# tum-pbs/differentiable-piso

Hardware: AMD Instinct MI355X
Metric: PISO steps/s (fwd+adjoint) at 2048^2 staggered grid (higher is better)
Workload: dtype f64

## Files before the change

### differentiable-piso_amd/csrc/cg.hip

```cpp
#include <atomic>
#include "cg_kernels.h"
#include "cg_dispatch.h"
#include "cg_tiny.h"
#include "options.h"
#include <cstdio>
#include <vector>

namespace piso {

struct CgProfile {
  int enabled = 0, stride = 8;
  double ms[4] = {0, 0, 0, 0};
  long long count[4] = {0, 0, 0, 0};
};
static CgProfile g_prof;

struct HostPoll {
  CgState* pinned = nullptr;
  hipEvent_t ev[2] = {nullptr, nullptr};
  hipEvent_t seg_ev[2] = {nullptr, nullptr};
  int cus = 0;
};
static std::atomic<unsigned> g_persist_launches{0};
static int g_persist_fallbacks = 0;
static thread_local int tl_xcd_map[kPersistMaxGrid];
static thread_local int tl_xcd_map_n = 0;
static long long g_tiny_solves = 0;
enum { DI_PATH = 0, DI_SIZEOF_T, DI_SIZEOF_CT, DI_V, DI_RECON, DI_SYMMETRIC, DI_ROWS_PER_WAVE, DI_K1_GRID, DI_K1_TILES, DI_R, DI_NQ,
       DI_WAVES, DI_LAUNCH_GRID, DI_PADDED, DI_XCD_LOCAL, DI_FELL_BACK, DI_TINY_PER_X, DI_K2_GRID, DI_SEGMENTS, DI_COUNT };
static thread_local int tl_dispatch[DI_COUNT];
static thread_local int tl_dispatch_n = 0;
static bool g_xcd_local_failed = false;
static long long g_verify_runs = 0;
static int g_verify_failures = 0;
constexpr int kPollDevices = 16;
static thread_local HostPoll tl_poll_dev[kPollDevices];
static thread_local HostPoll* tl_poll_cur = &tl_poll_dev[0];
#define tl_poll (*tl_poll_cur)

static int ensure_poll() {
  int dev = 0;
  PISO_HIP_CHECK(hipGetDevice(&dev));
  if (dev < 0 || dev >= kPollDevices) { set_error_msg("piso_cg_solve: device ordinal out of range"); return PISO_ERR_INVALID_ARG; }
  tl_poll_cur = &tl_poll_dev[dev];
  if (!tl_poll.pinned) {
    PISO_HIP_CHECK(hipHostMalloc(reinterpret_cast<void**>(&tl_poll.pinned), 2 * sizeof(CgState), hipHostMallocDefault));
    PISO_HIP_CHECK(hipEventCreateWithFlags(&tl_poll.ev[0], hipEventDisableTiming));
    PISO_HIP_CHECK(hipEventCreateWithFlags(&tl_poll.ev[1], hipEventDisableTiming));
    PISO_HIP_CHECK(hipDeviceGetAttribute(&tl_poll.cus, hipDeviceAttributeMultiprocessorCount, dev));
  }
  return PISO_OK;
}

constexpr size_t kPadMaxCells = (size_t)1 << 19;
static bool padded_dims(int nx, int ny, int per_x, int per_y, int elem, int* nxp, int* nyp) {
  *nxp = nx; *nyp = ny;
  if (elem != 8 || nx % 2 != 0 || nx < 8 || ny < 8) return false;
  const bool pad_x = nx % 128 != 0, pad_y = ny % 2 != 0;
  if (!pad_x && !pad_y) return false;
  const int px = (nx + 127) / 128 * 128;
  int py = (ny + 3) / 4 * 4;
  if (px != nx && per_x) return false;
  if (py != ny && per_y) {
    py = ny;
    if (ny % 2 != 0 || ((long long)(px / 128) * (ny / 2)) % 2 != 0) return false;
  }
  if ((size_t)px * py > kPadMaxCells) return false;
  *nxp = px; *nyp = py;
  return true;
}

template <typename T>
static size_t cg_workspace_bytes(int nx_in, int ny_in) {
  int nx = nx_in, ny = ny_in;
  const bool padded = padded_dims(nx_in, ny_in, 0, 0, (int)sizeof(T), &nx, &ny);
  const size_t n = (size_t)nx * ny + (padded ? 2 * (size_t)nx * ny : 0);
  size_t b = 0;
  b += 11 * align_up(n * sizeof(T), 256);
  b += align_up(4 * n * sizeof(float), 256) + 256;
  b += 3 * align_up(3 * kMaxPartials * sizeof(T), 256);
  b += align_up(SC_COUNT * sizeof(T), 256) + align_up(2 * sizeof(CgState), 256) + 512;
  b += align_up(kPersistWsWordsAll * sizeof(unsigned), 256);
  return b + 4096;
}

static void record_dispatch(int path, size_t state_bytes, size_t coef_bytes, int tiny_per_x, int V = 0, bool recon = false, bool symmetric = false,
                            const CgTiling* t = nullptr, const PersistPlan* p = nullptr, bool fell_back = false) {
  int* d = tl_dispatch;
  for (int i = 0; i < DI_COUNT; ++i) d[i] = 0;
  d[DI_PATH] = path; d[DI_SIZEOF_T] = (int)state_bytes; d[DI_SIZEOF_CT] = (int)coef_bytes; d[DI_TINY_PER_X] = tiny_per_x;
  d[DI_V] = V; d[DI_RECON] = recon ? 1 : 0; d[DI_SYMMETRIC] = symmetric ? 1 : 0; d[DI_FELL_BACK] = fell_back ? 1 : 0;
  if (t) { d[DI_ROWS_PER_WAVE] = t->rows_per_wave; d[DI_K1_GRID] = t->g1; d[DI_K1_TILES] = t->k1_tiles; d[DI_K2_GRID] = t->g2; }
  if (p) d[DI_PADDED] = p->ragged ? 1 : 0;
  if (p && p->R) { d[DI_R] = p->R; d[DI_NQ] = p->NQ; d[DI_WAVES] = p->waves; d[DI_LAUNCH_GRID] = p->launch_grid; d[DI_XCD_LOCAL] = p->xcd_local ? 1 : 0; }
  tl_dispatch_n = DI_COUNT;
}

struct EventPool {
  static constexpr int kMax = 64;
// ... 11 lines not shown
      PISO_HIP_CHECK(hipEventCreate(&ep.start[q][i]));
      PISO_HIP_CHECK(hipEventCreate(&ep.stop[q][i]));
    }
  ep.created = true;
  return PISO_OK;
}

static int read_profile(const EventPool& ep, const SegmentTimes& seg, float* kernel_ms_out) {
  double ms[2] = {0, 0};
  for (int q = 0; q < 2; ++q)
    for (int i = 0; i < ep.used[q]; ++i) {
      float t = 0;
      PISO_HIP_CHECK(hipEventElapsedTime(&t, ep.start[q][i], ep.stop[q][i]));
      ms[q] += t;
    }
  if (kernel_ms_out) {
    kernel_ms_out[0] = ep.used[0] ? (float)(ms[0] / ep.used[0]) : 0.f;
    kernel_ms_out[1] = ep.used[1] ? (float)(ms[1] / ep.used[1]) : 0.f;
  }
  if (g_prof.enabled) {
    for (int q = 0; q < 2; ++q) { g_prof.ms[q] += ms[q]; g_prof.count[q] += ep.used[q]; }
    g_prof.ms[2] += seg.ms; g_prof.count[2] += seg.iters; g_prof.count[3] += seg.launches;
  }
  if (kernel_ms_out && seg.iters > 0) { kernel_ms_out[0] = (float)(seg.ms / seg.iters); kernel_ms_out[1] = 0.f; }
  return PISO_OK;
}

struct PersistTiming {
  unsigned long long* ticks = nullptr;
  ~PersistTiming() { if (ticks) (void)hipFree(ticks); }
};
static int print_persist_timing(const unsigned long long* ticks, int grid, int k_last) {
  std::vector<unsigned long long> h(12 * grid);
  PISO_HIP_CHECK(hipMemcpy(h.data(), ticks, h.size() * sizeof(unsigned long long), hipMemcpyDeviceToHost));
  const char* names[9] = {"D (p update, stencil, sums, publish)", "exchange", "U (stencil, x / r update, ring)", "-", "-",
                           "  exchange: wave sums + drain of the perimeter stores", "  exchange: first barrier", "  exchange: publish + polling",
                           "  exchange: record sums + second barrier"};
  const double f = 0.01 / (double)(k_last > 0 ? k_last : 1);
  if (opt(OPT_CG_PERSIST_TIMING) >= 2) {
    for (int b = 0; b < grid; ++b)
      fprintf(stderr, "cg_persist_wg %3d xcd %d band %3d  D %.2f  exchange %.2f  U %.2f  | drain %.2f  barrier1 %.2f  publish+poll %.2f  sums %.2f\n", b, (int)h[9 * grid + b], (int)h[10 * grid + b],
              f * (double)h[0 * grid + b], f * (double)h[1 * grid + b], f * (double)h[2 * grid + b],
              f * (double)h[5 * grid + b], f * (double)h[6 * grid + b], f * (double)h[7 * grid + b], f * (double)h[8 * grid + b]);
  }
  for (int q = 0; q < 9; ++q) {
    double s = 0, mn = 1e300, mx = 0;
    for (int b = 0; b < grid; ++b) { const double v = (double)h[q * grid + b]; s += v; mn = v < mn ? v : mn; mx = v > mx ? v : mx; }
    fprintf(stderr, "cg_persist %s: avg %.2f us/iter  min %.2f  max %.2f\n", names[q], f * s / grid, f * mn, f * mx);
  }
  return PISO_OK;
}

template <typename T, typename CT>
static int verify_residual(const CgArgs<T>& a, const PersistCtl& pc, hipStream_t stream, bool* failed) {
  unsigned* out2 = reinterpret_cast<unsigned*>(pc.err) + 4;
  PISO_HIP_CHECK(hipMemsetAsync(out2, 0, 2 * sizeof(unsigned), stream));
  const int gvf = grid_for((long long)a.nx * a.ny, kBlock * 4, 1024);
  cg_verify_sum_x<T><<<gvf, kBlock, 0, stream>>>(a, a.partsA);
  cg_verify_gap<T, CT><<<gvf, kBlock, 0, stream>>>(a, a.partsA, gvf, out2);
  PISO_LAUNCH_CHECK();
  unsigned h2[2] = {0, 0};
  PISO_HIP_CHECK(hipMemcpyAsync(h2, out2, sizeof(h2), hipMemcpyDeviceToHost, stream));
  PISO_HIP_CHECK(hipStreamSynchronize(stream));
  float gap, scale;
  memcpy(&gap, &h2[0], 4); memcpy(&scale, &h2[1], 4);
  ++g_verify_runs;
  *failed = (gap > 1e-5f * scale && gap > 1e-30f) || opt(OPT_CG_VERIFY) == 2;
  return PISO_OK;
}

static int inspect_poll(int slot, int* stop_it) {
  hipError_t e = hipEventSynchronize(tl_poll.ev[slot]);
  if (e != hipSuccess) { set_error("hipEventSynchronize", e); return -1; }
  if (tl_poll.pinned[slot].done) { *stop_it = tl_poll.pinned[slot].iterations; return 1; }
  return 0;
}
static int poll_batch(size_t n) {
  const double t_iter_us = (double)n * 120.0 / 4.0e6;
  const int batch = (int)(1000.0 / (t_iter_us < 8.0 ? 8.0 : t_iter_us));
  return batch < 10 ? 10 : (batch > 200 ? 200 : batch);
}

template <typename T, typename CT, int V, bool RECON>
static int cg_run(CgArgs<T> a, unsigned* persist_ws, bool symmetric, float accuracy, int max_iterations, int rank_deficient, int reset, int fixed,
                  int* iterations_out, float* kernel_ms_out, hipStream_t stream, bool allow_persist) {
  const size_t n = (size_t)a.nx * a.ny;
  const CgTiling tile = cg_tile(a, V, opt(OPT_CG_RPW), opt(OPT_CG_MAXBLOCKS));
  const int g1 = tile.g1, g2 = tile.g2, gflat = tile.gflat;
  a.accuracy = fixed ? -1.0f : accuracy;

  { const int rc = ensure_poll(); if (rc != PISO_OK) return rc; }
  const bool prof = (kernel_ms_out != nullptr) || g_prof.enabled;
  EventPool& ep = tl_events;
  if (prof) { const int rc = ensure_events(ep); if (rc != PISO_OK) return rc; }
  ep.used[0] = ep.used[1] = 0;
  const int prof_stride = g_prof.stride > 0 ? g_prof.stride : 8;

  cg_init<T><<<gflat, kBlock, 0, stream>>>(a, rank_deficient);
  PISO_LAUNCH_CHECK();

  const int batch = poll_batch(n);
  int sv = 0, polls = 0, stop_it = -1;
  const int total = fixed ? fixed : max_iterations;
  bool finished = false;
  bool pending = false;
  int k_last = -1;
  PersistPlan plan = persist_plan(PersistQuery{a.nx, a.ny, V, a.per_y, a.nx_true != 0, sizeof(T), sizeof(CT), RECON, symmetric, false, tl_poll.cus,
                                               opt(OPT_CG_PERSIST), opt(OPT_CG_PERSIST_R), opt(OPT_CG_PERSIST_HALF), opt(OPT_CG_PERSIST_NQ),
                                               opt(OPT_CG_XCD_LOCAL), g_xcd_local_failed, allow_persist});
  PersistCtl pc;
  { const int rc = persist_prepare<T, CT, RECON, false>(plan, tl_poll.cus, pc, persist_ws, stream); if (rc != PISO_OK) return rc; }
  PersistTiming timing;
  if (plan.R && kPersistDiag && opt_on(OPT_CG_PERSIST_TIMING)) {
    PISO_HIP_CHECK(hipMalloc(reinterpret_cast<void**>(&timing.ticks), 12 * plan.launch_grid * sizeof(unsigned long long)));
    PISO_HIP_CHECK(hipMemsetAsync(timing.ticks, 0, 12 * plan.launch_grid * sizeof(unsigned long long), stream));
    pc.timing = timing.ticks;
  }
  record_dispatch(plan.R ? 3 : 2, sizeof(T), sizeof(CT), 0, V, RECON, symmetric, &tile, &plan, !allow_persist);
  const int seg_len = persist_segment_len(n, opt(OPT_CG_SEGMENT));
  hipEvent_t* seg_ev = tl_poll.seg_ev;
  if (plan.R && prof && !seg_ev[0]) { PISO_HIP_CHECK(hipEventCreate(&seg_ev[0])); PISO_HIP_CHECK(hipEventCreate(&seg_ev[1])); }
  SegmentTimes seg;
  int segments_run = 0, unsynced = 0;
  for (int k = 0; k < total && !finished; ++k) {
    const bool is_reset = !fixed && ((k + 1) % reset == 0);
    if (plan.R && k > 0 && !is_reset) {
      int ke = total;
      if (!fixed) { const int next_reset = ((k + 1 + reset - 1) / reset) * reset - 1; if (next_reset < ke) ke = next_reset; }
      if (ke > k + seg_len) ke = k + seg_len;
      if (ke > k) {
        if (prof) PISO_HIP_CHECK(hipEventRecord(seg_ev[0], stream));
        { const int rc = persist_launch<T, CT, RECON, false>(plan, a, pc, g_persist_launches.fetch_add(1, std::memory_order_relaxed), k, ke, sv, pending, NoSlab{}, stream);
          if (rc != PISO_OK) return rc; }
        if (prof) PISO_HIP_CHECK(hipEventRecord(seg_ev[1], stream));
        const bool defer = !prof && ke - k <= 32 && unsynced + (ke - k) <= 256 && ke < total;
        unsynced = defer ? unsynced + (ke - k) : 0;
        if (!defer) {
          PISO_HIP_CHECK(hipMemcpyAsync(&tl_poll.pinned[0], &a.state[0], sizeof(CgState), hipMemcpyDeviceToHost, stream));
          int herr = 0;
          PISO_HIP_CHECK(hipMemcpyAsync(&herr, pc.err, sizeof(int), hipMemcpyDeviceToHost, stream));
          PISO_HIP_CHECK(hipStreamSynchronize(stream));
          if (herr) {
            ++g_persist_fallbacks;
            if (plan.xcd_local) g_xcd_local_failed = true;
            return kPersistRetry;
          }
          if (prof) {
            const int ran = tl_poll.pinned[0].done ? (tl_poll.pinned[0].iterations - k > 0 ? tl_poll.pinned[0].iterations - k : 0) : ke - k;
            float t = 0; PISO_HIP_CHECK(hipEventElapsedTime(&t, seg_ev[0], seg_ev[1])); seg.ms += t; seg.iters += ran < ke - k ? ran : ke - k; ++seg.launches;
          }
          if (tl_poll.pinned[0].done) { finished = true; stop_it = tl_poll.pinned[0].iterations; }
        }
        ++segments_run;
        k_last = ke - 1;
        pending = false;
        k = ke - 1;
        continue;
      }
    }
    const bool sample = prof && (k % prof_stride == prof_stride - 1) && ep.used[0] < EventPool::kMax && !is_reset && k > 0;
    if (is_reset) {
      if (pending) { cg_flush_x<T><<<gflat, kBlock, 0, stream>>>(a, k - 1, sv); pending = false; }
      cg_k1<T, CT, V, RECON><<<g1, kBlock, 0, stream>>>(a, k, MODE_RESET, sv, k > 0 ? 1 : 0, 0);
      ++sv;
      cg_reset_residual<T><<<gflat, kBlock, 0, stream>>>(a, sv);
      cg_k1<T, CT, V, RECON><<<g1, kBlock, 0, stream>>>(a, k, MODE_INIT, sv, 0, 0);
    } else if (k == 0) {
      cg_k1<T, CT, V, RECON><<<g1, kBlock, 0, stream>>>(a, k, MODE_INIT, sv, 0, 0);
    } else {
      if (sample) PISO_HIP_CHECK(hipEventRecord(ep.start[0][ep.used[0]], stream));
      cg_k1<T, CT, V, RECON><<<g1, kBlock, 0, stream>>>(a, k, MODE_NORMAL, sv, 1, pending ? 1 : 0);
      if (sample) PISO_HIP_CHECK(hipEventRecord(ep.stop[0][ep.used[0]++], stream));
      ++sv;
    }
    if (sample) PISO_HIP_CHECK(hipEventRecord(ep.start[1][ep.used[1]], stream));
    cg_k2<T, V><<<g2, kBlock, 0, stream>>>(a, k, sv);
    if (sample) PISO_HIP_CHECK(hipEventRecord(ep.stop[1][ep.used[1]++], stream));
    PISO_LAUNCH_CHECK();
    pending = true;
    k_last = k;
    if (!fixed && ((k + 1) % batch == 0) && k + 1 < total) {
      const int slot = polls & 1;
      PISO_HIP_CHECK(hipMemcpyAsync(&tl_poll.pinned[slot], &a.state[sv & 1], sizeof(CgState), hipMemcpyDeviceToHost, stream));
      PISO_HIP_CHECK(hipEventRecord(tl_poll.ev[slot], stream));
      if (polls > 0) {
        const int r = inspect_poll((polls - 1) & 1, &stop_it);
        if (r < 0) return PISO_ERR_HIP;
        if (r > 0) finished = true;
      }
      ++polls;
    }
  }
  if (pending && k_last >= 0) cg_flush_x<T><<<gflat, kBlock, 0, stream>>>(a, k_last, sv);
  if (!fixed && !finished) {
    const int slot = polls & 1;
    PISO_HIP_CHECK(hipMemcpyAsync(&tl_poll.pinned[slot], &a.state[sv & 1], sizeof(CgState), hipMemcpyDeviceToHost, stream));
    PISO_HIP_CHECK(hipEventRecord(tl_poll.ev[slot], stream));
    const int r = inspect_poll(slot, &stop_it);
    if (r < 0) return PISO_ERR_HIP;
    if (r > 0) finished = true;
  }
  PISO_HIP_CHECK(hipStreamSynchronize(stream));
  if (opt(OPT_CG_XCD_MAP) == 1) {
    tl_xcd_map_n = 0;
    if (segments_run > 0 && !plan.xcd_local && plan.grid <= kPersistMaxGrid) {
      PISO_HIP_CHECK(hipMemcpy(tl_xcd_map, pc.xcd + kPersistXcdTable, (size_t)plan.grid * sizeof(int), hipMemcpyDeviceToHost));
      tl_xcd_map_n = plan.grid;
    }
  }
  if (segments_run > 0) {
    int herr = 0;
    PISO_HIP_CHECK(hipMemcpy(&herr, pc.err, sizeof(int), hipMemcpyDeviceToHost));
    if (herr) { ++g_persist_fallbacks; return kPersistRetry; }
  }
  if (segments_run > 0 && sizeof(T) == 8 && !fixed && opt(OPT_CG_VERIFY) != 0) {
    bool failed = false;
    { const int rc = verify_residual<T, CT>(a, pc, stream, &failed); if (rc != PISO_OK) return rc; }
    if (failed) { ++g_verify_failures; ++g_persist_fallbacks; return kPersistRetry; }
  }
  if (timing.ticks) { const int rc = print_persist_timing(timing.ticks, plan.grid, k_last); if (rc != PISO_OK) return rc; }
  if (iterations_out) *iterations_out = finished ? stop_it : total;
  tl_dispatch[DI_SEGMENTS] = segments_run;
  return prof ? read_profile(ep, seg, kernel_ms_out) : PISO_OK;
}

template <typename T>
__global__ __launch_bounds__(kBlock) void cg_copy_rows(const T* __restrict__ src, T* __restrict__ dst, int nx, int ny, int ld_src, int ld_dst) {
  const size_t n = (size_t)nx * ny;
  for (size_t i = (size_t)blockIdx.x * kBlock + threadIdx.x; i < n; i += (size_t)gridDim.x * kBlock) {
    const size_t j = i / (size_t)nx, c = i % (size_t)nx;
    dst[j * (size_t)ld_dst + c] = src[j * (size_t)ld_src + c];
  }
}

template <typename T>
static int cg_solve(int nx, int ny, int per_x, int per_y, const T* L, const T* b, T* x_out, float accuracy,
                    int max_iterations, int rank_deficient, int reset, int fixed, int* iterations_out,
                    float* kernel_ms_out, void* ws, size_t ws_bytes, piso_stream_t stream_, int* iterations_dev = nullptr) {
  tl_dispatch_n = 0;
  if (nx < 1 || ny < 1 || !L || !b || !x_out || !ws || max_iterations < 0 || reset < 1) {
    set_error_msg("piso_cg_solve: invalid argument");
    return PISO_ERR_INVALID_ARG;
  }
  if (ws_bytes < cg_workspace_bytes<T>(nx, ny)) {
    set_error_msg("piso_cg_solve: workspace too small");
    return PISO_ERR_INVALID_ARG;
  }
  hipStream_t stream = static_cast<hipStream_t>(stream_);
  const size_t n_true = (size_t)nx * ny;
  if (n_true <= (size_t)kTinyMaxCells && opt(OPT_CG_TINY) != 0 && opt(OPT_CG_PERSIST) < 0) {
    CgState* st_dev = reinterpret_cast<CgState*>(ws);
    const int total = fixed ? fixed : max_iterations;
    hipEvent_t* ev = nullptr;
    if (kernel_ms_out) {
      { const int rc = ensure_poll(); if (rc != PISO_OK) return rc; }
      ev = tl_poll.seg_ev;
      if (!ev[0]) { PISO_HIP_CHECK(hipEventCreate(&ev[0])); PISO_HIP_CHECK(hipEventCreate(&ev[1])); }
      PISO_HIP_CHECK(hipEventRecord(ev[0], stream));
    }
    const bool async = iterations_dev != nullptr;
    const bool cols = nx <= 64 && ny <= kColsMaxNy && (!per_x || nx == 64) && opt(OPT_CG_TINY) != 2;
    if (cols && per_x)
      cg_tiny_cols<T, true><<<1, kTinyThreads, 0, stream>>>(L, b, x_out, nx, ny, per_y, fixed ? -1.0f : accuracy, total, fixed ? 0 : reset,
                                                            rank_deficient, st_dev, iterations_dev);
    else if (cols)
      cg_tiny_cols<T, false><<<1, kTinyThreads, 0, stream>>>(L, b, x_out, nx, ny, per_y, fixed ? -1.0f : accuracy, total, fixed ? 0 : reset,
                                                             rank_deficient, st_dev, iterations_dev);
    else
      cg_tiny<T><<<1, kTinyThreads, 0, stream>>>(L, b, x_out, nx, ny, per_x, per_y, fixed ? -1.0f : accuracy, total, fixed ? 0 : reset,
                                                 rank_deficient, st_dev, iterations_dev);
    PISO_LAUNCH_CHECK();
    ++g_tiny_solves;
// ... 173 lines not shown
```

### differentiable-piso_amd/csrc/cg_kernels.h

```cpp
#pragma once
#include <stdlib.h>

#include "piso_common.h"

namespace piso {

struct CgState {
  int flag;
  int done;
  int iterations;
  int pad;
};

enum { MODE_NORMAL = 0, MODE_INIT = 1, MODE_RESET = 2 };
enum { SC_C = 0, SC_PZ = 1, SC_VS = 2, SC_ALPHA = 3, SC_COUNT = 8 };

template <typename T>
struct CgArgs {
  const T* cC;
  const void *oS, *oW, *oE, *oN;
  const T* b;
  T *x, *r, *z;
  T* p[2];
  T* zp[2];
  T* partsA;
  T* partsB;
  T* partsS;
  T* scal;
  CgState* state;
  int nx, ny, per_x, per_y;
  const T* gA;
  const T* gB;
  int ntx, nty, rows_per_wave;
  int nA, nB;
  float accuracy;
  int nt;
  int nx_true, ny_true;
  double ncells;
};
template <typename T>
__device__ __forceinline__ bool true_cell(const CgArgs<T>& a, size_t i) {
  if (!a.nx_true) return true;
  return (int)(i % (size_t)a.nx) < a.nx_true && (int)(i / (size_t)a.nx) < a.ny_true;
}

template <typename T, int V>
struct Vec {
  T v[V];
};

template <typename S, int V>
__device__ __forceinline__ Vec<S, V> ldc(const S* __restrict__ p) {
  Vec<S, V> o;
  constexpr int B = sizeof(S) * V;
  using raw4 = __attribute__((ext_vector_type(4))) unsigned int;
  using raw2 = __attribute__((ext_vector_type(2))) unsigned int;
  if constexpr (B % 16 == 0) {
#pragma unroll
    for (int q = 0; q < B / 16; ++q) {
      const raw4 t = reinterpret_cast<const raw4*>(p)[q];
      __builtin_memcpy(reinterpret_cast<char*>(&o) + 16 * q, &t, 16);
    }
  } else if constexpr (B == 8) {
    const raw2 t = *reinterpret_cast<const raw2*>(p);
    __builtin_memcpy(&o, &t, 8);
  } else {
    static_assert(V == 1, "unsupported vector width");
    o.v[0] = p[0];
  }
  return o;
}
template <typename T, int V>
__device__ __forceinline__ Vec<T, V> ldv(const T* __restrict__ p) { return ldc<T, V>(p); }

template <typename S, int V>
__device__ __forceinline__ Vec<S, V> ldc_nt(const S* __restrict__ p) {
  Vec<S, V> o;
  constexpr int B = sizeof(S) * V;
  using raw4 = __attribute__((ext_vector_type(4))) unsigned int;
  using raw2 = __attribute__((ext_vector_type(2))) unsigned int;
  if constexpr (B % 16 == 0) {
#pragma unroll
    for (int q = 0; q < B / 16; ++q) {
      const raw4 t = __builtin_nontemporal_load(reinterpret_cast<const raw4*>(p) + q);
      __builtin_memcpy(reinterpret_cast<char*>(&o) + 16 * q, &t, 16);
    }
  } else if constexpr (B == 8) {
    const raw2 t = __builtin_nontemporal_load(reinterpret_cast<const raw2*>(p));
    __builtin_memcpy(&o, &t, 8);
  } else {
    o.v[0] = __builtin_nontemporal_load(p);
  }
// ... 93 lines not shown
    for (int e = 0; e < V; ++e) { o.s.v[e] = 0; o.q.v[e] = 0; }
    if (!active) return o;
    if (a.per_y != 2) {
      if (j < 0) { if (!a.per_y) return o; j = ny - 1; }
      if (j >= ny) { if (!a.per_y) return o; j = 0; }
    }
    const ptrdiff_t i = (ptrdiff_t)j * nx + c0;
    o.s = ldv<T, V>(src + i);
    if (use_pin) o.q = ldv<T, V>(pin + i);
    return o;
  };

  const CgState st = a.state[sv & 1];
  const T sc_pz = a.scal[SC_PZ], sc_vs = a.scal[SC_VS], sc_alpha = a.scal[SC_ALPHA];
  const int ntiles = a.ntx * a.nty;
  const XcdRange tr = xcd_range(ntiles);
  const int dir = (wave & 1) ? -1 : 1;
  auto tile_geom = [&](int t, int& jb, int& je, int& c0, bool& active) {
    const int ty = t / a.ntx, tx = t - ty * a.ntx;
    jb = (ty * 4 + wave) * a.rows_per_wave;
    je = min(jb + a.rows_per_wave, ny);
    c0 = (tx * 64 + lane) * V;
    active = c0 < nx;
  };
  Raw rawB, rawC;
  {
    int jb, je, c0; bool active;
    if (tr.begin < tr.end) {
      tile_geom(tr.begin, jb, je, c0, active);
      if (jb < ny) {
        const int j = (dir > 0) ? jb : je - 1;
        rawB = load_raw(j - dir, c0, active);
        rawC = load_raw(j, c0, active);
      }
    }
  }

  T beta = 0;
  CgState nst = st;
  if (do_check) {
    T pb[3];
    prologue_reduce<T, 3>(a.partsB, a.nB, a.gB, pb, smem);
    if (!st.done) {
      if (k > 0 && (k % 5) == 0) {
        const int exceeded = pb[2] > 0;
        if (st.flag && !exceeded) { nst.done = 1; nst.iterations = k; }
        else nst.flag = 1;
      }
      if (mode == MODE_NORMAL) beta = -(pb[0] + sc_vs * pb[1]) / sc_pz;
    }
  }
  if (mode == MODE_RESET && !nst.done) nst.flag = 0;
  if (writes_state && blockIdx.x == 0 && threadIdx.x == 0) a.state[(sv + 1) & 1] = nst;
  if (st.done) return;
  const T alpha_prev = pending ? sc_alpha : (T)0;
  const bool only_flush = nst.done;

  auto combine = [&](const Raw& w) -> Vec<T, V> {
    Vec<T, V> o = w.s;
    if (use_pin) {
#pragma unroll
      for (int e = 0; e < V; ++e) o.v[e] = fma(beta, w.q.v[e], o.v[e]);
    }
    return o;
  };
  auto val_at = [&](int j, int c) -> T {
    if (a.per_y != 2) {
      if (j < 0) { if (!a.per_y) return (T)0; j = ny - 1; }
      if (j >= ny) { if (!a.per_y) return (T)0; j = 0; }
    }
    const ptrdiff_t i = (ptrdiff_t)j * nx + c;
    T v = src[i];
    if (use_pin) v = fma(beta, pin[i], v);
    return v;
  };

  T acc_p = 0, acc_pr = 0, acc_pz = 0;
  for (int t = tr.begin; t < tr.end; t += tr.step) {
    int jb, je, c0; bool active;
    tile_geom(t, jb, je, c0, active);
    if (jb >= ny) continue;
    if (only_flush) {
      if (active && pending && use_pin)
        for (int j = jb; j < je; ++j) {
          const size_t i = (size_t)j * nx + c0;
          Vec<T, V> xv = ldv<T, V>(a.x + i);
          const Vec<T, V> q = ldv<T, V>(pin + i);
#pragma unroll
          for (int e = 0; e < V; ++e) xv.v[e] = fma(alpha_prev, q.v[e], xv.v[e]);
          stv<T, V>(a.x + i, xv);
        }
      continue;
    }
    int j = (dir > 0) ? jb : je - 1;
    if (t != tr.begin) {
      rawB = load_raw(j - dir, c0, active);
      rawC = load_raw(j, c0, active);
    }
    Vec<T, V> behind = combine(rawB);
    Vec<T, V> cur = combine(rawC);
    Vec<T, V> praw = rawC.q;
    if (a.per_y == 2 && active && mode != MODE_RESET && (j - dir < 0 || j - dir >= ny))
      stv<T, V>(pout + (ptrdiff_t)(j - dir) * nx + c0, behind);
    for (int cnt = jb; cnt < je; ++cnt, j += dir) {
      const Raw rawA = load_raw(j + dir, c0, active);
      const Vec<T, V> ahead = combine(rawA);
      if (a.per_y == 2 && active && mode != MODE_RESET && (j + dir < 0 || j + dir >= ny))
// ... 51 lines not shown
          tmp = fma((T)kE.v[e], pe, tmp);
          tmp = fma((T)kN.v[e], pnn, tmp);
          zz.v[e] = tmp;
          acc_p += cur.v[e];
          acc_pr = fma(cur.v[e], rr.v[e], acc_pr);
          acc_pz = fma(cur.v[e], tmp, acc_pz);
        }
        if (a.nt & 4) { stv_nt<T, V>(a.z + i, zz); if (mode != MODE_RESET) stv_nt<T, V>(pout + i, cur); }
        else { stv<T, V>(a.z + i, zz); if (mode != MODE_RESET) stv<T, V>(pout + i, cur); }
      }
      behind = cur;
      cur = ahead;
      praw = rawA.q;
      rawC = rawA;
    }
  }
  if (only_flush) return;
  T part[3] = {acc_p, acc_pr, acc_pz};
  block_sum<T, 3>(part, smem);
  if (threadIdx.x == 0) {
#pragma unroll
    for (int q = 0; q < 3; ++q) a.partsA[q * kMaxPartials + blockIdx.x] = part[q];
  }
}

template <typename T, int V>
__global__ __launch_bounds__(kBlock) void cg_k2(CgArgs<T> a, int k, int sv) {
  __shared__ T smem[16];
  constexpr int D = 4;
  const T* __restrict__ zp = a.z;
  T* __restrict__ rp = a.r;
  const size_t n = (size_t)a.nx * a.ny;
  const int nchunks = (int)((n / V + kBlock - 1) / kBlock);
  const XcdRange cr = xcd_range(nchunks);
  const CgState st = a.state[sv & 1];
  const T sc_c = a.scal[SC_C];
  Vec<T, V> zq[D], rq[D];
  size_t iq[D];
  bool okq[D];
  int ch = cr.begin;
#pragma unroll
  for (int d = 0; d < D; ++d) {
    const int c = ch + d * cr.step;
    iq[d] = ((size_t)c * kBlock + threadIdx.x) * V;
    okq[d] = c < cr.end && iq[d] < n;
    if (okq[d]) {
      if (a.nt & 2) { zq[d] = ldc_nt<T, V>(zp + iq[d]); rq[d] = ldc_nt<T, V>(rp + iq[d]); }
      else { zq[d] = ldv<T, V>(zp + iq[d]); rq[d] = ldv<T, V>(rp + iq[d]); }
    }
  }

  T pa[3];
  prologue_reduce<T, 3>(a.partsA, a.nA, a.gA, pa, smem);
  if (st.done) return;
  const T vs = sc_c * pa[0];
  const T pz = pa[2] + vs * pa[0];
  T alpha = 0;
  if (absval(pz) > 0) alpha = pa[1] / pz;
  if (blockIdx.x == 0 && threadIdx.x == 0) { a.scal[SC_PZ] = pz; a.scal[SC_VS] = vs; a.scal[SC_ALPHA] = alpha; }

  T acc_rz = 0, acc_r = 0, acc_ex = 0;
  const T accuracy = (T)a.accuracy;
  while (ch < cr.end) {
#pragma unroll
    for (int d = 0; d < D; ++d) {
      if (okq[d]) {
        Vec<T, V> r0 = rq[d];
#pragma unroll
        for (int e = 0; e < V; ++e) {
          r0.v[e] = fma(-alpha, zq[d].v[e] + (true_cell(a, iq[d] + e) ? vs : (T)0), r0.v[e]);
          acc_rz = fma(r0.v[e], zq[d].v[e], acc_rz);
          acc_r += r0.v[e];
          acc_ex += (absval(r0.v[e]) < accuracy) ? (T)0 : (T)1;
        }
        if (a.nt & 1) stv_nt<T, V>(rp + iq[d], r0); else stv<T, V>(rp + iq[d], r0);
      }
      const int c = ch + (d + D) * cr.step;
      iq[d] = ((size_t)c * kBlock + threadIdx.x) * V;
      okq[d] = c < cr.end && iq[d] < n;
      if (okq[d]) {
        if (a.nt & 2) { zq[d] = ldc_nt<T, V>(zp + iq[d]); rq[d] = ldc_nt<T, V>(rp + iq[d]); }
        else { zq[d] = ldv<T, V>(zp + iq[d]); rq[d] = ldv<T, V>(rp + iq[d]); }
      }
    }
    ch += D * cr.step;
  }
  T part[3] = {acc_rz, acc_r, acc_ex};
  block_sum<T, 3>(part, smem);
  if (threadIdx.x == 0) {
#pragma unroll
    for (int q = 0; q < 3; ++q) a.partsB[q * kMaxPartials + blockIdx.x] = part[q];
  }
}

template <typename T>
__global__ __launch_bounds__(kBlock) void cg_flush_x(CgArgs<T> a, int k_last, int sv) {
  if (a.state[sv & 1].done) return;
  const T alpha = a.scal[SC_ALPHA];
  const T* __restrict__ p = a.p[(k_last + 1) & 1];
  const size_t n = (size_t)a.nx * a.ny;
  for (size_t i = (size_t)blockIdx.x * kBlock + threadIdx.x; i < n; i += (size_t)gridDim.x * kBlock)
    a.x[i] = fma(alpha, p[i], a.x[i]);
}

template <typename T>
__global__ __launch_bounds__(kBlock) void cg_reset_residual(CgArgs<T> a, int sv) {
  __shared__ T smem[16];
  if (a.state[sv & 1].done) return;
  T pa[1];
  reduce_partials<T, 1>(a.partsA, a.nA, pa, smem);
  if (a.gA) pa[0] = a.gA[0];
  const T vs = a.scal[SC_C] * pa[0];
  const size_t n = (size_t)a.nx * a.ny;
  for (size_t i = (size_t)blockIdx.x * kBlock + threadIdx.x; i < n; i += (size_t)gridDim.x * kBlock)
    a.r[i] = a.b[i] - (a.z[i] + (true_cell(a, i) ? vs : (T)0));
}

template <typename T>
__global__ __launch_bounds__(kBlock) void cg_setup_coeffs(const T* __restrict__ L, T* cC, T* oT, float* oF, T* parts,
                                                           int* flags, size_t n, int nx = 0, int ny = 0, int per_x = 0,
                                                           int per_y = 0, int ldx = 0, size_t n_out = 0) {
  __shared__ T smem[16];
  T acc = 0;
  bool bad = false, bad_recon = false, bad_sym = (nx == 0);
  for (size_t i = (size_t)blockIdx.x * kBlock + threadIdx.x; i < n; i += (size_t)gridDim.x * kBlock) {
    const T* row = L + i * 5;
    if (nx > 0) {
      const int ci = (int)(i % (size_t)nx), cj = (int)(i / (size_t)nx);
      const T e_nb = (ci + 1 < nx) ? L[(i + 1) * 5 + 1] : (per_x ? L[(i - (size_t)(nx - 1)) * 5 + 1] : (T)0);
      const T n_nb = (cj + 1 < ny) ? L[(i + (size_t)nx) * 5 + 0] : (per_y == 1 ? L[(size_t)ci * 5 + 0] : (per_y == 2 ? row[4] : (T)0));
      bad_sym |= !(row[3] == e_nb) || !(row[4] == n_nb);
    }
    const T o[4] = {row[0], row[1], row[3], row[4]};
    const size_t io = ldx ? (i / (size_t)nx) * (size_t)ldx + (i % (size_t)nx) : i;
    const size_t no = ldx ? n_out : n;
    cC[io] = row[2];
#pragma unroll
    for (int q = 0; q < 4; ++q) {
      const float f = (float)o[q];
      oT[q * no + io] = o[q];
      oF[q * no + io] = f;
      bad |= !((T)f == o[q]);
    }
    T d = 0;
    d -= (T)(float)o[0]; d -= (T)(float)o[3]; d -= (T)(float)o[1]; d -= (T)(float)o[2];
    bad_recon |= !(d == row[2]);
    acc += absval(row[2]);
  }
  if (bad) flags[0] = 1;
  if (bad_recon) flags[1] = 1;
  if (bad_sym) flags[2] = 1;
  T part[1] = {acc};
  block_sum<T, 1>(part, smem);
  if (threadIdx.x == 0) parts[blockIdx.x] = part[0];
}

template <typename T>
__global__ __launch_bounds__(kBlock) void cg_init(CgArgs<T> a, int rank_deficient, const T* global_diag_sum = nullptr,
                                                   double global_cells = 0) {
  __shared__ T smem[16];
  T pa[1];
// ... 78 lines not shown
```

### differentiable-piso_amd/csrc/cg_persist1.h

```cpp
#pragma once
#include <cstddef>
#include <type_traits>

#include "cg_persist.h"
#include "peer.h"

namespace piso {

struct NoSlab {};
struct SlabCtl {
  PeerView pv;
  double ncells;
  char *rows_own, *rows_lo, *rows_hi;
  unsigned hop_ticks;
};
template <typename T, typename SL>
struct Persist1Kargs { CgArgs<T> a; PersistCtl c; int k_begin, k_end, sv, pend; SL sl; };
template <typename F>
__device__ __forceinline__ F karg(unsigned off) {
  typedef __attribute__((address_space(4))) const char kchar;
  typedef __attribute__((address_space(4))) const unsigned kword;
  kchar* kp = (kchar*)__builtin_amdgcn_kernarg_segment_ptr();
  asm volatile("" : "+s"(kp));
  static_assert(sizeof(F) % 4 == 0, "whole dwords");
// ... 459 lines not shown
    switch (j) {
      case 15: return ring;
      case 14: return dpp_mov32<0x111>(ring); case 13: return dpp_mov32<0x112>(ring); case 12: return dpp_mov32<0x113>(ring);
      case 11: return dpp_mov32<0x114>(ring); case 10: return dpp_mov32<0x115>(ring); case 9: return dpp_mov32<0x116>(ring);
      case 8: return dpp_mov32<0x117>(ring); case 7: return dpp_mov32<0x118>(ring); case 6: return dpp_mov32<0x119>(ring);
      case 5: return dpp_mov32<0x11a>(ring); case 4: return dpp_mov32<0x11b>(ring); case 3: return dpp_mov32<0x11c>(ring);
      case 2: return dpp_mov32<0x11d>(ring); case 1: return dpp_mov32<0x11e>(ring); default: return dpp_mov32<0x11f>(ring);
    }
  }
}
template <bool UP, typename S>
__device__ __forceinline__ S shift_ring(S v, S ring, int j) {
  constexpr int ctrl = UP ? 0x138  : 0x130 ;
  if constexpr (sizeof(S) == 8) {
    const unsigned long long b = (unsigned long long)__double_as_longlong((double)v), e = (unsigned long long)__double_as_longlong((double)ring);
    const int elo = ring_to_end32<UP>((int)(unsigned)e, j), ehi = ring_to_end32<UP>((int)(unsigned)(e >> 32), j);
    const unsigned lo = (unsigned)__builtin_amdgcn_update_dpp(elo, (int)(unsigned)b, ctrl, 0xf, 0xf, false);
    const unsigned hi = (unsigned)__builtin_amdgcn_update_dpp(ehi, (int)(unsigned)(b >> 32), ctrl, 0xf, 0xf, false);
    return (S)__longlong_as_double((long long)(((unsigned long long)hi << 32) | lo));
  } else {
    const int e = ring_to_end32<UP>(__float_as_int((float)ring), j);
    return (S)__int_as_float(__builtin_amdgcn_update_dpp(e, __float_as_int((float)v), ctrl, 0xf, 0xf, false));
  }
}
__device__ __forceinline__ void ring_lane(int lane, int R, int& side, int& er) {
  side = (lane < R) ? 0 : ((lane >= 48 && lane < 48 + R) ? 1 : 2);
  er = (side == 1) ? lane - 48 : lane;
}

constexpr int kSystem = 17;

template <typename T, typename CT, int R, int NQ, bool RECON, bool SYM, bool SLAB = false, bool RAGGED = false, bool LOCAL = false>
__global__ __launch_bounds__(kPersistThreads) void cg_persist1(CgArgs<T> a, PersistCtl c, int k_begin, int k_end, int sv, int pend,
                                                               std::conditional_t<SLAB, SlabCtl, NoSlab> sl = {}) {
  static_assert(!(SLAB && RAGGED), "a slab is never padded");
  static_assert(!(SLAB && LOCAL), "a slab's neighbours are other GPUs");
  constexpr int kPub = LOCAL ? kPlain : kAgent;
  constexpr int kHalo = kAgent;
  constexpr int V = 16 / sizeof(T);
  static_assert(R * NQ <= 16 && 2 * R <= 64, "at most 16 rows per wave; the edge columns of a region fit one wave-wide load");
  static_assert(!SLAB || sizeof(T) == 8, "mailbox rows hold 8-byte elements");
  __shared__ T xs[kPersistWaves * NQ * R * 64 * V];
  __shared__ T smem[2 * kX1Sm + (SLAB ? 2 * kX1SmX : 0)];
  constexpr bool kParkHalos = (NQ * R < 16) || NQ == 1;
  __shared__ T halo_s[kParkHalos ? kPersistWaves * NQ * 2 * 64 * V : 1];
  constexpr bool kRingLds = sizeof(CT) == 4;
  constexpr bool kParkRing = kRingLds;
  constexpr int kRingBytes = 64 * (int)sizeof(T) + 64 * (int)sizeof(CT) + (kParkRing ? 64 * (int)sizeof(T) : 0);
  constexpr unsigned kRingR = 64u * (unsigned)sizeof(T) + 64u * (unsigned)sizeof(CT);
  __shared__ __attribute__((aligned(16))) unsigned char ring_s[kRingLds ? kPersistWaves * NQ * kRingBytes : 16];
  const int nx = a.nx, ny = a.ny;
  const int lane = threadIdx.x & 63;
  const int wave = __builtin_amdgcn_readfirstlane(threadIdx.x >> 6);
  int wg = blockIdx.x;
  if (gridDim.x % kXcds == 0) wg = (blockIdx.x % kXcds) * (gridDim.x / kXcds) + blockIdx.x / kXcds;
  int nslots = (int)gridDim.x;
  if constexpr (LOCAL) {
    __shared__ int local_rank_s;
    if (threadIdx.x == 0) {
      const int xcc = (int)(__builtin_amdgcn_s_getreg(20 | (0 << 6) | (3 << 11)) & 7);
      const int arrival = __hip_atomic_fetch_add(c.xcd + xcc, 1, __ATOMIC_RELAXED, __HIP_MEMORY_SCOPE_AGENT);
      int rank = -1;
      if (arrival < c.local_n) {
        if (arrival == c.local_n - 1) {
          int none = 0;
          __hip_atomic_compare_exchange_strong(c.xcd + 8, &none, xcc + 1, __ATOMIC_RELAXED, __ATOMIC_RELAXED, __HIP_MEMORY_SCOPE_AGENT);
        }
        int winner = 0;
        unsigned spins = 0;
        while ((winner = __hip_atomic_load(c.xcd + 8, __ATOMIC_RELAXED, __HIP_MEMORY_SCOPE_AGENT)) == 0) {
          if (++spins > (1u << 22)) break;
          __builtin_amdgcn_s_sleep(2);
        }
        if (winner == xcc + 1) rank = arrival;
        else if (winner == 0) { *c.err = 1; }
      }
      local_rank_s = rank;
    }
    __syncthreads();
    wg = __builtin_amdgcn_readfirstlane(local_rank_s);
    if (wg < 0) return;
    nslots = c.local_n;
  }
  const int slot = LOCAL ? wg : (int)blockIdx.x;
  constexpr bool kHier = !LOCAL;
  static_assert(!SLAB || kHier, "the node level of the slab instance rides on the tree exchange");
  unsigned hx = 0;
  constexpr bool kLocalAll = LOCAL;
  __shared__ int hier_s[(kHier || kLocalAll) ? 4 : 1];
  if constexpr (kLocalAll) { if (threadIdx.x == 0) hier_s[2] = 0; }
  if constexpr (kHier) {
    hx = hier_enter(c, hier_s);
    if (hier_s[1]) return;
  }
  int j0[NQ], tx0[NQ];
  bool has[NQ];
#pragma unroll
  for (int q = 0; q < NQ; ++q) {
    const int reg = (wg * c.waves + wave) * NQ + q;
    has[q] = wave < c.waves && reg < c.nreg;
    const int ty = has[q] ? reg / c.ntx : 0;
    tx0[q] = has[q] ? reg - ty * c.ntx : 0;
    j0[q] = ty * R;
  }
  const unsigned nbytesT = (unsigned)((size_t)nx * ny * sizeof(T)), nbytesC = (unsigned)((size_t)nx * ny * sizeof(CT));
  const unsigned rowT = (unsigned)(nx * sizeof(T)), rowC = (unsigned)(nx * sizeof(CT));
// ... 626 lines not shown
```

Baseline: 5.282.

## Make persistent CG segment checks asynchronous with device-side error early-exit

Replaces the blocking stream synchronize after each persistent CG segment with double-buffered pinned-memory status copies and events that are inspected one segment behind. Kernels now check a device error flag (and the done state) and return early, so segments launched speculatively after a failure or convergence do little work. Residual verification is enqueued before the final synchronize instead of adding its own sync. The host stops blocking between segments, at the cost of possibly launching an extra segment and more complex error and retry handling.

```diff
diff --git a/differentiable-piso_amd/csrc/cg.hip b/differentiable-piso_amd/csrc/cg.hip
--- a/differentiable-piso_amd/csrc/cg.hip
+++ b/differentiable-piso_amd/csrc/cg.hip
@@ -17,6 +17,8 @@
 
 struct HostPoll {
   CgState* pinned = nullptr;
+  int* err = nullptr;
+  unsigned* gap = nullptr;
   hipEvent_t ev[2] = {nullptr, nullptr};
   hipEvent_t seg_ev[2] = {nullptr, nullptr};
   int cus = 0;
@@ -44,7 +46,9 @@
   if (dev < 0 || dev >= kPollDevices) { set_error_msg("piso_cg_solve: device ordinal out of range"); return PISO_ERR_INVALID_ARG; }
   tl_poll_cur = &tl_poll_dev[dev];
   if (!tl_poll.pinned) {
-    PISO_HIP_CHECK(hipHostMalloc(reinterpret_cast<void**>(&tl_poll.pinned), 2 * sizeof(CgState), hipHostMallocDefault));
+    PISO_HIP_CHECK(hipHostMalloc(reinterpret_cast<void**>(&tl_poll.pinned), 2 * sizeof(CgState) + 4 * sizeof(int), hipHostMallocDefault));
+    tl_poll.err = reinterpret_cast<int*>(tl_poll.pinned + 2);
+    tl_poll.gap = reinterpret_cast<unsigned*>(tl_poll.err + 2);
     PISO_HIP_CHECK(hipEventCreateWithFlags(&tl_poll.ev[0], hipEventDisableTiming));
     PISO_HIP_CHECK(hipEventCreateWithFlags(&tl_poll.ev[1], hipEventDisableTiming));
     PISO_HIP_CHECK(hipDeviceGetAttribute(&tl_poll.cus, hipDeviceAttributeMultiprocessorCount, dev));
@@ -162,26 +166,34 @@
 }
 
 template <typename T, typename CT>
-static int verify_residual(const CgArgs<T>& a, const PersistCtl& pc, hipStream_t stream, bool* failed) {
+static int verify_residual(const CgArgs<T>& a, const PersistCtl& pc, hipStream_t stream) {
   unsigned* out2 = reinterpret_cast<unsigned*>(pc.err) + 4;
   PISO_HIP_CHECK(hipMemsetAsync(out2, 0, 2 * sizeof(unsigned), stream));
   const int gvf = grid_for((long long)a.nx * a.ny, kBlock * 4, 1024);
   cg_verify_sum_x<T><<<gvf, kBlock, 0, stream>>>(a, a.partsA);
   cg_verify_gap<T, CT><<<gvf, kBlock, 0, stream>>>(a, a.partsA, gvf, out2);
   PISO_LAUNCH_CHECK();
-  unsigned h2[2] = {0, 0};
-  PISO_HIP_CHECK(hipMemcpyAsync(h2, out2, sizeof(h2), hipMemcpyDeviceToHost, stream));
-  PISO_HIP_CHECK(hipStreamSynchronize(stream));
+  PISO_HIP_CHECK(hipMemcpyAsync(tl_poll.gap, out2, 2 * sizeof(unsigned), hipMemcpyDeviceToHost, stream));
+  return PISO_OK;
+}
+static bool verify_failed() {
   float gap, scale;
-  memcpy(&gap, &h2[0], 4); memcpy(&scale, &h2[1], 4);
+  memcpy(&gap, &tl_poll.gap[0], 4); memcpy(&scale, &tl_poll.gap[1], 4);
   ++g_verify_runs;
-  *failed = (gap > 1e-5f * scale && gap > 1e-30f) || opt(OPT_CG_VERIFY) == 2;
-  return PISO_OK;
-}
-
+  return (gap > 1e-5f * scale && gap > 1e-30f) || opt(OPT_CG_VERIFY) == 2;
+}
+
+static int place_look(int slot, const CgState* st, const int* err, hipStream_t stream) {
+  PISO_HIP_CHECK(hipMemcpyAsync(&tl_poll.pinned[slot], st, sizeof(CgState), hipMemcpyDeviceToHost, stream));
+  if (err) PISO_HIP_CHECK(hipMemcpyAsync(&tl_poll.err[slot], err, sizeof(int), hipMemcpyDeviceToHost, stream));
+  else tl_poll.err[slot] = 0;
+  PISO_HIP_CHECK(hipEventRecord(tl_poll.ev[slot], stream));
+  return PISO_OK;
+}
 static int inspect_poll(int slot, int* stop_it) {
   hipError_t e = hipEventSynchronize(tl_poll.ev[slot]);
   if (e != hipSuccess) { set_error("hipEventSynchronize", e); return -1; }
+  if (tl_poll.err[slot]) return -2;
   if (tl_poll.pinned[slot].done) { *stop_it = tl_poll.pinned[slot].iterations; return 1; }
   return 0;
 }
@@ -210,7 +222,7 @@
   PISO_LAUNCH_CHECK();
 
   const int batch = poll_batch(n);
-  int sv = 0, polls = 0, stop_it = -1;
+  int sv = 0, stop_it = -1;
   const int total = fixed ? fixed : max_iterations;
   bool finished = false;
   bool pending = false;
@@ -232,6 +244,31 @@
   if (plan.R && prof && !seg_ev[0]) { PISO_HIP_CHECK(hipEventCreate(&seg_ev[0])); PISO_HIP_CHECK(hipEventCreate(&seg_ev[1])); }
   SegmentTimes seg;
   int segments_run = 0, unsynced = 0;
+  a.err = pc.err;
+  int looks = 0, inspected = 0, seg_looks = 0;
+  struct { int kb, ke; bool timed; } look_seg[2] = {{0, 0, false}, {0, 0, false}};
+  auto inspect_upto = [&](int upto) -> int {
+    for (; inspected < upto; ++inspected) {
+      const int slot = inspected & 1;
+      const int r = inspect_poll(slot, &stop_it);
+      if (r == -1) return PISO_ERR_HIP;
+      if (r == -2) {
+        ++g_persist_fallbacks;
+        if (plan.xcd_local) g_xcd_local_failed = true;
+        PISO_HIP_CHECK(hipStreamSynchronize(stream));
+        return kPersistRetry;
+      }
+      if (look_seg[slot].timed) {
+        const CgState& hs = tl_poll.pinned[slot];
+        const int kb = look_seg[slot].kb, len = look_seg[slot].ke - kb;
+        const int ran = hs.done ? (hs.iterations - kb > 0 ? hs.iterations - kb : 0) : len;
+        float t = 0; PISO_HIP_CHECK(hipEventElapsedTime(&t, seg_ev[0], seg_ev[1])); seg.ms += t; seg.iters += ran < len ? ran : len; ++seg.launches;
+        look_seg[slot].timed = false;
+      }
+      if (r > 0) finished = true;
+    }
+    return PISO_OK;
+  };
   for (int k = 0; k < total && !finished; ++k) {
     const bool is_reset = !fixed && ((k + 1) % reset == 0);
     if (plan.R && k > 0 && !is_reset) {
@@ -246,20 +283,13 @@
         const bool defer = !prof && ke - k <= 32 && unsynced + (ke - k) <= 256 && ke < total;
         unsynced = defer ? unsynced + (ke - k) : 0;
         if (!defer) {
-          PISO_HIP_CHECK(hipMemcpyAsync(&tl_poll.pinned[0], &a.state[0], sizeof(CgState), hipMemcpyDeviceToHost, stream));
-          int herr = 0;
-          PISO_HIP_CHECK(hipMemcpyAsync(&herr, pc.err, sizeof(int), hipMemcpyDeviceToHost, stream));
-          PISO_HIP_CHECK(hipStreamSynchronize(stream));
-          if (herr) {
-            ++g_persist_fallbacks;
-            if (plan.xcd_local) g_xcd_local_failed = true;
-            return kPersistRetry;
-          }
-          if (prof) {
-            const int ran = tl_poll.pinned[0].done ? (tl_poll.pinned[0].iterations - k > 0 ? tl_poll.pinned[0].iterations - k : 0) : ke - k;
-            float t = 0; PISO_HIP_CHECK(hipEventElapsedTime(&t, seg_ev[0], seg_ev[1])); seg.ms += t; seg.iters += ran < ke - k ? ran : ke - k; ++seg.launches;
-          }
-          if (tl_poll.pinned[0].done) { finished = true; stop_it = tl_poll.pinned[0].iterations; }
+          const int slot = looks & 1;
+          look_seg[slot].kb = k; look_seg[slot].ke = ke; look_seg[slot].timed = prof;
+          { const int rc = place_look(slot, &a.state[sv & 1], pc.err, stream); if (rc != PISO_OK) return rc; }
+          ++looks;
+          const int behind = (prof || seg_looks == 0) ? 0 : 1;
+          ++seg_looks;
+          { const int rc = inspect_upto(looks - behind); if (rc != PISO_OK) return rc; }
         }
         ++segments_run;
         k_last = ke - 1;
@@ -289,28 +319,21 @@
     PISO_LAUNCH_CHECK();
     pending = true;
     k_last = k;
-    if (!fixed && ((k + 1) % batch == 0) && k + 1 < total) {
-      const int slot = polls & 1;
-      PISO_HIP_CHECK(hipMemcpyAsync(&tl_poll.pinned[slot], &a.state[sv & 1], sizeof(CgState), hipMemcpyDeviceToHost, stream));
-      PISO_HIP_CHECK(hipEventRecord(tl_poll.ev[slot], stream));
-      if (polls > 0) {
-        const int r = inspect_poll((polls - 1) & 1, &stop_it);
-        if (r < 0) return PISO_ERR_HIP;
-        if (r > 0) finished = true;
-      }
-      ++polls;
+    if (!fixed && ((k + 1) % batch == 0) && k + 1 < total && segments_run == 0) {
+      { const int rc = place_look(looks & 1, &a.state[sv & 1], pc.err, stream); if (rc != PISO_OK) return rc; }
+      ++looks;
+      { const int rc = inspect_upto(looks - 1); if (rc != PISO_OK) return rc; }
     }
   }
   if (pending && k_last >= 0) cg_flush_x<T><<<gflat, kBlock, 0, stream>>>(a, k_last, sv);
-  if (!fixed && !finished) {
-    const int slot = polls & 1;
-    PISO_HIP_CHECK(hipMemcpyAsync(&tl_poll.pinned[slot], &a.state[sv & 1], sizeof(CgState), hipMemcpyDeviceToHost, stream));
-    PISO_HIP_CHECK(hipEventRecord(tl_poll.ev[slot], stream));
-    const int r = inspect_poll(slot, &stop_it);
-    if (r < 0) return PISO_ERR_HIP;
-    if (r > 0) finished = true;
-  }
+  if ((!fixed && !finished) || segments_run > 0) {
+    { const int rc = place_look(looks & 1, &a.state[sv & 1], pc.err, stream); if (rc != PISO_OK) return rc; }
+    ++looks;
+  }
+  const bool verify = segments_run > 0 && sizeof(T) == 8 && !fixed && opt(OPT_CG_VERIFY) != 0;
+  if (verify) { const int rc = verify_residual<T, CT>(a, pc, stream); if (rc != PISO_OK) return rc; }
   PISO_HIP_CHECK(hipStreamSynchronize(stream));
+  { const int rc = inspect_upto(looks); if (rc != PISO_OK) return rc; }
   if (opt(OPT_CG_XCD_MAP) == 1) {
     tl_xcd_map_n = 0;
     if (segments_run > 0 && !plan.xcd_local && plan.grid <= kPersistMaxGrid) {
@@ -318,16 +341,7 @@
       tl_xcd_map_n = plan.grid;
     }
   }
-  if (segments_run > 0) {
-    int herr = 0;
-    PISO_HIP_CHECK(hipMemcpy(&herr, pc.err, sizeof(int), hipMemcpyDeviceToHost));
-    if (herr) { ++g_persist_fallbacks; return kPersistRetry; }
-  }
-  if (segments_run > 0 && sizeof(T) == 8 && !fixed && opt(OPT_CG_VERIFY) != 0) {
-    bool failed = false;
-    { const int rc = verify_residual<T, CT>(a, pc, stream, &failed); if (rc != PISO_OK) return rc; }
-    if (failed) { ++g_verify_failures; ++g_persist_fallbacks; return kPersistRetry; }
-  }
+  if (verify && verify_failed()) { ++g_verify_failures; ++g_persist_fallbacks; return kPersistRetry; }
   if (timing.ticks) { const int rc = print_persist_timing(timing.ticks, plan.grid, k_last); if (rc != PISO_OK) return rc; }
   if (iterations_out) *iterations_out = finished ? stop_it : total;
   tl_dispatch[DI_SEGMENTS] = segments_run;
diff --git a/differentiable-piso_amd/csrc/cg_kernels.h b/differentiable-piso_amd/csrc/cg_kernels.h
--- a/differentiable-piso_amd/csrc/cg_kernels.h
+++ b/differentiable-piso_amd/csrc/cg_kernels.h
@@ -37,7 +37,10 @@
   int nt;
   int nx_true, ny_true;
   double ncells;
+  const int* err = nullptr;
 };
+template <typename T>
+__device__ __forceinline__ bool solve_failed(const CgArgs<T>& a) { return a.err && *a.err != 0; }
 template <typename T>
 __device__ __forceinline__ bool true_cell(const CgArgs<T>& a, size_t i) {
   if (!a.nx_true) return true;
@@ -237,7 +240,7 @@
   }
   if (mode == MODE_RESET && !nst.done) nst.flag = 0;
   if (writes_state && blockIdx.x == 0 && threadIdx.x == 0) a.state[(sv + 1) & 1] = nst;
-  if (st.done) return;
+  if (st.done || solve_failed(a)) return;
   const T alpha_prev = pending ? sc_alpha : (T)0;
   const bool only_flush = nst.done;
 
@@ -395,7 +398,7 @@
 
   T pa[3];
   prologue_reduce<T, 3>(a.partsA, a.nA, a.gA, pa, smem);
-  if (st.done) return;
+  if (st.done || solve_failed(a)) return;
   const T vs = sc_c * pa[0];
   const T pz = pa[2] + vs * pa[0];
   T alpha = 0;
@@ -438,7 +441,7 @@
 
 template <typename T>
 __global__ __launch_bounds__(kBlock) void cg_flush_x(CgArgs<T> a, int k_last, int sv) {
-  if (a.state[sv & 1].done) return;
+  if (a.state[sv & 1].done || solve_failed(a)) return;
   const T alpha = a.scal[SC_ALPHA];
   const T* __restrict__ p = a.p[(k_last + 1) & 1];
   const size_t n = (size_t)a.nx * a.ny;
@@ -449,7 +452,7 @@
 template <typename T>
 __global__ __launch_bounds__(kBlock) void cg_reset_residual(CgArgs<T> a, int sv) {
   __shared__ T smem[16];
-  if (a.state[sv & 1].done) return;
+  if (a.state[sv & 1].done || solve_failed(a)) return;
   T pa[1];
   reduce_partials<T, 1>(a.partsA, a.nA, pa, smem);
   if (a.gA) pa[0] = a.gA[0];
diff --git a/differentiable-piso_amd/csrc/cg_persist1.h b/differentiable-piso_amd/csrc/cg_persist1.h
--- a/differentiable-piso_amd/csrc/cg_persist1.h
+++ b/differentiable-piso_amd/csrc/cg_persist1.h
@@ -535,6 +535,9 @@
   const int nx = a.nx, ny = a.ny;
   const int lane = threadIdx.x & 63;
   const int wave = __builtin_amdgcn_readfirstlane(threadIdx.x >> 6);
+  if constexpr (!SLAB) {
+    if (__hip_atomic_load(c.err, __ATOMIC_RELAXED, __HIP_MEMORY_SCOPE_AGENT) != 0 || a.state[sv & 1].done) return;
+  }
   int wg = blockIdx.x;
   if (gridDim.x % kXcds == 0) wg = (blockIdx.x % kXcds) * (gridDim.x / kXcds) + blockIdx.x / kXcds;
   int nslots = (int)gridDim.x;
```

New measurement: 5.183, median of 2. 0.981x the previous value.
